# ssteinberg/wave_tracer

Hardware: AMD Instinct MI355X
Metric: Msamples/sec (whole node), cornell-box 1440^2 wave-mode (higher is better)
Workload: dtype f32

## Files before the change

### wave_tracer_amd/csrc/kernels_trace.hip

```cpp
#include "wtgpu_kernels.h"

namespace wtk {

}
#include "kernels_trace_refill.h"
namespace wtk {

__global__ void __launch_bounds__(kBlock, WTGPU_LB_TRACE) k_trace_refill(launch_args_t a, int in, int first_round, uint32_t round) { trace_refill_body(a, in, first_round, round); }

#ifndef WTGPU_SM_EXACT_MIN
#define WTGPU_SM_EXACT_MIN 24
#endif
#ifndef WTGPU_SM_SPLIT_NODE
#define WTGPU_SM_SPLIT_NODE 0
#endif
#ifndef WTGPU_SM_BOTH
#define WTGPU_SM_BOTH 0
#endif
enum : int { PH_IDLE = 0, PH_NODE = 1, PH_TRI = 2, PH_EXACT = 3, PH_SERVE = 4, PH_POLICY = 5, PH_RAYDONE = 6 };
#ifdef WTGPU_SM_PROF
#define SP_DECL() unsigned long long sp_t[8] = {0, 0, 0, 0, 0, 0, 0, 0}, sp_l[8] = {0, 0, 0, 0, 0, 0, 0, 0}, sp_n[8] = {0, 0, 0, 0, 0, 0, 0, 0}; long long sp_c = 0
#define SP_BEGIN() sp_c = clock64()
#define SP_END(i, mask) do { const long long d_ = clock64() - sp_c; sp_t[i] += (unsigned long long)d_; sp_l[i] += (unsigned long long)d_ * (unsigned long long)__popcll(mask); sp_n[i] += 1; } while (0)
#else
// ... 608 lines not shown
            uint32_t* slot = a.st.tris + (size_t)w * kTriListWords;
            const uint_list_t tris{slot, 1u, (a.collect_list & 1u) ? kMaxConeTris : 0u, reinterpret_cast<float*>(slot + kMaxConeTris)};
            cone_query_t q;
            for (;;) {
                const int need = aw_next(a.sc, ts.env, rt, stack, ts.aw, q, r);
                if (need == AW_FINAL) break;
                if (need == AW_TEST) {
                    aw_test_done(ts.aw, cone_attempt_too_short_by(a.sc, ts.env, ts.aw.cand, ts.aw.sr, ts.aw.min_df_prog));
                    continue;
                }
                while (cq_running(q)) {
                    while (q.s > 0 && q.leaf == 0) cq_node_step(ns, ts.env, stack, q);
                    if (q.leaf != 0) cq_leaf_step(a.sc, ts.env, stack, tris, q);
                }
                cq_end(ts.env, tris, q);
                if (aw_query_done(a.sc, ts.env, ts.aw, q.rec, r)) break;
            }
        }
        tr_finish(a, ctl, ctr, have, w, r);
    }
    if (a.count_stats) flush_counters(a.st.counters, ctr);
}

__global__ void __launch_bounds__(64, WTGPU_LB_HEAVY) k_trace_heavy(launch_args_t a) {
    __shared__ coop_shared_t sh;
    coop_set_dropped_counter(sh, a.st.counters + kDroppedSlot);
    uint32_t* ctl = a.st.ctl;
    const uint32_t n = ctl[CTL_HEAVY_COUNT];
    const uint32_t* hq = a.st.heavy_queue;
    uint32_t* head = ctl + CTL_HEAVY_HEAD;
    bdpt_counters_t ctr;
    memset(&ctr, 0, sizeof(ctr));
    const size_t W2 = 2 * (size_t)a.st.cap;
    const bool rt = a.sc.sensor.ray_trace_only || a.sc.opts.force_ray_tracing;
    for (;;) {
        const uint32_t item = wave_grab_item(head);
        if (item >= n) break;
        const uint32_t w = hq[item];
        const walk_trace_in_t wk = walk_load_trace_in(a.st.walks, a.st.walk_words, w);
        const uint_list_t tris{a.st.tris + (size_t)w * kTriListWords, 1u, (a.collect_list & 1u) ? kMaxConeTris : 0u};
        const cone_t env = walk_trace_envelope(a.sc, wk);
        unsigned long long prof[12] = {0, 0, 0, 0, 0, 0, 0, 0, 0, 0, 0, 0};
        const long long tt0 = a.profile == 2 ? clock64() : 0;
        const float dist0 = __uint_as_float(a.st.trav[(size_t)w * kTravWords + WT_TRAV_WORD(dist)]);
        const uint32_t seg0 = a.st.trav[(size_t)w * kTravWords + WT_TRAV_WORD(ntris)];
        const uint32_t nray0 = a.st.trav[(size_t)w * kTravWords + WT_TRAV_WORD(n_ray_queries)], ncone0 = a.st.trav[(size_t)w * kTravWords + WT_TRAV_WORD(n_cone_queries)];
        ray_hit_t axis;
        axis.tuid = a.st.trav[(size_t)w * kTravWords + WT_TRAV_WORD(tuid)];
        axis.bx = __uint_as_float(a.st.trav[(size_t)w * kTravWords + WT_TRAV_WORD(bx)]);
        axis.by = __uint_as_float(a.st.trav[(size_t)w * kTravWords + WT_TRAV_WORD(by)]);
        axis.dist = __uint_as_float(a.st.trav[(size_t)w * kTravWords + WT_TRAV_WORD(pdist)]);
        axis.front_face = a.st.trav[(size_t)w * kTravWords + WT_TRAV_WORD(front_face)];
        const uint32_t short0 = a.st.trav[(size_t)w * kTravWords + WT_TRAV_WORD(overflow)];
        const trav_result_t tr2 = coop_traverse(a.sc, env, wavenum_to_wavelen_m(wk.k), WT_INF, rt, sh, tris, a.profile == 2 ? prof : nullptr, true, seg0, dist0, nray0, ncone0,
                                                &axis, !(a.collect_list & 1u) || (a.collect_list & 2u), a.heavy_probe != 0, a.heavy_cache ? short0 : kInvalid, a.heavy_cache ? wk.prev_offset_tuid : kInvalid, a.heavy_cache != 0);
        if (a.profile == 2 && threadIdx.x == 0) {
            prof[3] = (unsigned long long)(clock64() - tt0);
            for (int q = 0; q < 4; ++q) atomicAdd(a.st.counters + kNumCounters + q, prof[q]);
            atomicAdd(a.st.counters + kNumCounters + 5, prof[5]);
            atomicAdd(a.st.counters + kNumCounters + 6, prof[6]);
            atomicAdd(a.st.counters + kNumCounters + 7, prof[7]);
            for (int q = 8; q < 12; ++q) atomicAdd(a.st.counters + kNumCounters + q, prof[q]);
            atomicAdd(a.st.counters + kNumCounters + 4, 1ull);
        }
        if (threadIdx.x == 0) {
            soa_store(a.st.trav, kTravWords, w, tr2);
            ctr.segments += 1;
            ctr.ray_queries += tr2.n_ray_queries;
            ctr.cone_queries += tr2.n_cone_queries;
            if (a.collect_list & 1u) ctr.cone_tri_overflow += tr2.overflow;
        }
    }
    if (a.count_stats) flush_counters(a.st.counters, ctr);
}

__global__ void __launch_bounds__(256) k_calib_copy(const uint32_t* in, uint32_t* out, size_t n) {
    for (size_t i = blockIdx.x * (size_t)blockDim.x + threadIdx.x; i < n; i += (size_t)gridDim.x * blockDim.x) out[i] = in[i] + 1u;
}

__global__ void __launch_bounds__(kBlock) k_trace_rays(scene_t sc, const float* rays, uint32_t n, float* dist, uint32_t* tuid, float* bary, uint32_t* front) {
    __shared__ stack_entry_t lds[kLdsStack * kBlock];
    const uint32_t i = blockIdx.x * kBlock + threadIdx.x;
    if (i >= n) return;
    stack_entry_t spill[kSpillStack];
    stack_ref_t stack;
    lds_stack(lds, spill, stack);
    const float* r = rays + 8 * (size_t)i;
    ray_hit_t h;
    ads_intersect_ray(sc, vec3{r[0], r[1], r[2]}, vec3{r[3], r[4], r[5]}, range_t{r[6], r[7]}, stack, h);
    dist[i] = h.dist;
    tuid[i] = h.tuid;
    bary[2 * i] = h.bx;
    bary[2 * i + 1] = h.by;
    front[i] = h.front_face;
}
__global__ void __launch_bounds__(kBlock) k_traverse_cones(scene_t sc, const float* cones, uint32_t n, uint32_t cap, float* dist, uint32_t* flags,
// ... 22 lines not shown
            const uint32_t v = tris[j];
            uint32_t pos = m < cap ? m : cap;
            while (pos > 0 && out_tris[(size_t)i * cap + pos - 1] > v) {
                if (pos < cap) out_tris[(size_t)i * cap + pos] = out_tris[(size_t)i * cap + pos - 1];
                --pos;
            }
            if (pos < cap) out_tris[(size_t)i * cap + pos] = v;
            if (m < cap) ++m;
        }
    }
}

__global__ void __launch_bounds__(64) k_query_regions(scene_t sc, const float* cones, uint32_t n, uint32_t edge_cap, float* dist, uint32_t* flags,
                                                      uint32_t* primary, uint32_t* ntris, uint32_t* nedges, uint32_t* edges, float* flux, unsigned long long* dropped) {
    __shared__ coop_shared_t sh;
    __shared__ coop_gather_shared_t gsh;
    __shared__ coop_edges_t eg;
    coop_set_dropped_counter(sh, dropped);
    coop_set_dropped_counter(gsh, dropped);
    const uint32_t i = blockIdx.x;
    if (i >= n) return;
    const float* c = cones + 10 * (size_t)i;
    const vec3 d = normalize(vec3{c[3], c[4], c[5]});
    const cone_t env = make_cone(vec3{c[0], c[1], c[2]}, d, build_orthogonal_frame(d).t, c[6], c[8], c[7]);
    const uint_list_t none{nullptr, 1u, 0u};
    const trav_result_t tr = coop_traverse(sc, env, c[9], WT_INF, false, sh, none, nullptr, false, 0, 0.f, 0, 0, nullptr, true);
    uint32_t prim = kInvalid;
    gather_out_t ge{0.0, 0u, 0u, 0u}, gf{0.0, 0u, 0u, 0u};
    if (tr.ballistic) {
        prim = tr.tuid;
    } else if (!tr.empty) {
        const range_t izr{tr.dist, tr.dist + tr.region_depth};
        prim = tr.tuid;
        const vec2 ax = cone_axes(env, tr.dist);
        ge = coop_gather(sc, env, izr, env, cone_frame(env), izr, vec2{1.f, 1.f}, false, gsh, false, true, nullptr, 1, &eg);
        __syncthreads();
        if (sc.n_edges <= kCoopEdgeBits) {
            ge.n_edges = coop_edge_count(sc, eg);
            coop_edge_write(sc, eg, edges + (size_t)i * edge_cap, edge_cap);
        } else
            for (uint32_t j = threadIdx.x; j < ge.n_edges && j < edge_cap; j += 64) edges[(size_t)i * edge_cap + j] = eg.edge_ids[j];
        __syncthreads();
        gf = coop_gather(sc, env, izr, env, cone_frame(env), izr, vec2{ax.x / kBeamEnvelope, ax.y / kBeamEnvelope}, tr.front_face != 0, gsh, true, false);
    }
    if (threadIdx.x == 0) {
        dist[i] = tr.dist;
        flags[i] = (tr.empty ? 1u : 0u) | (tr.ballistic ? 2u : 0u) | (tr.front_face ? 4u : 0u);
        primary[i] = prim;
        ntris[i] = gf.n_tris;
// ... 7 lines not shown
```

### wave_tracer_amd/csrc/wt/coop.h

```cpp
#pragma once
#if defined(__HIPCC__)
#include "bvh.h"
#include "gauss.h"

namespace wt {

constexpr int kCoopStack = 512;
#ifndef WTGPU_COOP_LEAF_TRIS
#define WTGPU_COOP_LEAF_TRIS 256
#endif
constexpr uint32_t kCoopLeafTris = WTGPU_COOP_LEAF_TRIS;
constexpr uint32_t kCoopGatherLeafTris = 64;
constexpr uint32_t kCoopTriBuf = 64 + 8 * kCoopLeafTris;

#ifndef WTGPU_COOP_FLUSH_AT
#define WTGPU_COOP_FLUSH_AT 12
#endif
constexpr uint32_t kCoopFlushAt = WTGPU_COOP_FLUSH_AT;
constexpr uint32_t kCoopSurvCap = 128;

#ifndef WT_COOP_SPHERES
#define WT_COOP_SPHERES 1
#endif
#ifndef WT_COOP_SPHERE_PREFETCH
// ... 9 lines not shown
    float hit_dist[64];
};
struct coop_gather_shared_t {
    unsigned long long* dropped;
    stack_entry_t stack[kCoopStack];
    uint32_t tri_buf[64 + 8 * 64];
    uint32_t surv[kCoopSurvCap];
};
struct coop_edges_t {
    uint32_t edge_ids[96];
    uint32_t edge_bits[1024];
};
constexpr uint32_t kCoopEdgeBits = 32768;

template <class SH>
WT_D void coop_set_dropped_counter(SH& sh, unsigned long long* slot) {
    if (threadIdx.x == 0) sh.dropped = slot;
    __syncthreads();
}
WT_D float wave_min(float v) {
#pragma unroll
    for (int off = 32; off > 0; off >>= 1) v = fminf(v, __shfl_xor(v, off, 64));
    return v;
}

WT_D bool cone_child_test(const bvh8_node_t& n, int i, vec3 ro, vec3 rd, vec3 rinvd, bool sx, bool sy, bool sz, float ta, float ix,
                                       const range_t& range, float& tmin_out) {
    float ominx = n.minx[i] - ro.x, ominy = n.miny[i] - ro.y, ominz = n.minz[i] - ro.z;
    float omaxx = n.maxx[i] - ro.x, omaxy = n.maxy[i] - ro.y, omaxz = n.maxz[i] - ro.z;
    const bool outside = cone_box_outside(ominx, ominy, ominz, omaxx, omaxy, omaxz, rd, ta, ix, range);
    const float bx = sx ? ominx : omaxx, by = sy ? ominy : omaxy, bz = sz ? ominz : omaxz;
    const float dot_d_b = rd.x * bx + rd.y * by + rd.z * bz;
    const float maxz = clampf(dot_d_b, 0.f, range.max);
    const float enlr = fmaf(maxz, ta, ix);
    ominx -= enlr;
    ominy -= enlr;
    ominz -= enlr;
    omaxx += enlr;
    omaxy += enlr;
    omaxz += enlr;
    const float dminx = (sx ? omaxx : ominx) * rinvd.x, dmaxx = (sx ? ominx : omaxx) * rinvd.x;
    const float dminy = (sy ? omaxy : ominy) * rinvd.y, dmaxy = (sy ? ominy : omaxy) * rinvd.y;
    const float dminz = (sz ? omaxz : ominz) * rinvd.z, dmaxz = (sz ? ominz : omaxz) * rinvd.z;
    float tmin = 0.f, tmax = dmaxx;
    tmin = fmaxf_(tmin, dminx);
    tmax = fminf_(tmax, dmaxy);
    tmin = fmaxf_(tmin, dminy);
    tmax = fminf_(tmax, dmaxz);
    tmin = fmaxf_(tmin, dminz);
    tmin_out = tmin;
    return !outside && tmin <= tmax && tmax >= range.min && tmin <= range.max && !(tmin >= range.max);
}

template <bool any_hit>
WT_D bool coop_cone_query(const scene_t& sc, const cone_t& cone, const range_t& searchrange, float z_scale, coop_shared_t& sh,
                                       const uint_list_t& tris, cone_hit_t& rec, unsigned long long* prof = nullptr, float min_progress = -WT_INF) {
    const int lane = threadIdx.x & 63;
    const int grp = lane >> 3, sub = lane & 7;
    rec.dist = WT_INF;
    rec.front_face = 0;
    rec.ntris = 0;
    rec.overflow = 0;
    rec.aborted = 0;
    rec.too_short = 0;
    rec.short_tuid = kInvalid;
    if (sc.n_nodes == 0) return false;
    const vec3 ro = cone.o, rd = cone.d;
    const vec3 rinvd{1.f / rd.x, 1.f / rd.y, 1.f / rd.z};
    const bool sx = __builtin_signbit(rinvd.x), sy = __builtin_signbit(rinvd.y), sz = __builtin_signbit(rinvd.z);
    const float ta = cone.tan_alpha, ix = cone.x0;
    range_t range = any_hit ? searchrange : cone_search_range(cone, searchrange, rec.dist, z_scale);
    float slab_max = range.max;
    int s = 1;
    uint32_t leaf_total = 0, nsurv = 0;
    if (lane == 0) sh.stack[0] = stack_entry_t{0.f, 1};
    __syncthreads();
    auto compact = [&](float zmax) __attribute__((always_inline)) {
        if (rec.ntris == 0) return;
        __syncthreads();
        const bool mine = (uint32_t)lane < rec.ntris;
        const uint32_t val = mine ? tris[lane] : 0u;
        const float dv = mine ? sh.hit_dist[lane] : 0.f;
        const bool keep = mine && !(dv > zmax);
        const unsigned long long km = __ballot(keep);
        __syncthreads();
        if (keep) {
            const uint32_t np_ = (uint32_t)__popcll(km & ((1ull << lane) - 1ull));
            tris[np_] = val;
            sh.hit_dist[np_] = dv;
        }
        rec.ntris = (uint32_t)__popcll(km);
        __syncthreads();
    };
    auto flush = [&]() __attribute__((always_inline)) -> bool {
        __syncthreads();
        bool any = false;
        for (uint32_t b2 = 0; b2 < nsurv && !any; b2 += 64) {
#ifdef WTGPU_COOP_PROF
            if (prof) prof[9] += 1;
#endif
            const uint32_t k2 = b2 + lane;
            bool hit = false, ff = false;
            float d = WT_INF;
            uint32_t t2 = 0;
            if (k2 < nsurv) {
                t2 = sh.surv[k2];
                const tri_geo_t tri = sc.tri_geo[t2];
                ff = dot(tri.n, -rd) > 0.f;
                cone_tri_hit_t ht;
                if (intersect_cone_tri<any_hit>(cone, tri.a, tri.b, tri.c, tri.n, range, ht) && !(ht.dist > range.max)) {
                    hit = true;
                    d = ht.dist;
                }
            }
            const unsigned long long mask = __ballot(hit);
            if (!mask) continue;
            if (any_hit) {
                rec.short_tuid = (uint32_t)__shfl((int)t2, __ffsll((long long)mask) - 1, 64);
                any = true;
                break;
            }
            const float dm = wave_min(d);
            if (dm < rec.dist) {
                const unsigned long long m2 = __ballot(hit && d == dm);
                const int src = __ffsll((long long)m2) - 1;
                rec.front_face = (uint32_t)__shfl((int)ff, src, 64);
                rec.dist = dm;
                if (rec.dist - searchrange.min < min_progress) {
                    rec.short_tuid = (uint32_t)__shfl((int)t2, src, 64);
                    rec.too_short = 1;
                    any = true;
                    break;
                }
                range = cone_search_range(cone, searchrange, rec.dist, z_scale);
                slab_max = range.max;
                compact(slab_max);
            }
            const bool hit2 = hit && !(d > slab_max);
            const unsigned long long mask2 = __ballot(hit2);
            const uint32_t pos = rec.ntris + (uint32_t)__popcll(mask2 & ((1ull << lane) - 1ull));
            if (hit2 && pos < tris.cap) {
                tris[pos] = t2;
                sh.hit_dist[pos & 63u] = d;
            }
            const uint32_t total = rec.ntris + (uint32_t)__popcll(mask2);
            const uint32_t newn = total < tris.cap ? total : tris.cap;
            rec.overflow += total - newn;
            rec.ntris = newn;
            if (rec.overflow > 0) range.max = fminf_(range.max, rec.dist);
        }
        nsurv = 0;
        __syncthreads();
        return any;
    };
#ifdef WTGPU_COOP_PROF
    long long cp_t = clock64();
#define CP(k)                                              \
    do {                                                   \
        const long long n_ = clock64();                    \
        if (prof) prof[k] += (unsigned long long)(n_ - cp_t); \
        cp_t = n_;                                         \
    } while (0)
#else
#define CP(k) ((void)0)
#endif
    for (;;) {
        const long long ta0 = prof ? clock64() : 0;
        while (s > 0 && leaf_total < 64u) {
            const int np = s < 8 ? s : 8;
#ifndef WTGPU_COOP_PROF
            if (prof) prof[7] += 1ull + ((unsigned long long)np << 32);
#endif
// ... 30 lines not shown
            CP(1);
            const unsigned long long hm = __ballot(h);
            if (hm) {
                const uint32_t gbits = (uint32_t)(hm >> (grp * 8)) & 0xffu;
                int rank = 0;
#pragma unroll
                for (int j = 0; j < 8; ++j) {
                    const float tj = __shfl(tmin, (lane & ~7) + j, 64);
                    if (((gbits >> j) & 1u) && (tj > tmin || (tj == tmin && j < sub))) ++rank;
                }
                const int above = grp < 7 ? __popcll(hm >> ((grp + 1) * 8)) : 0;
                const int pos = s + above + rank;
                if (h && pos < kCoopStack) sh.stack[pos] = stack_entry_t{tmin, cp};
                else if (h) atomicAdd(sh.dropped, 1ull);
                const int total = s + __popcll(hm);
                s = total < kCoopStack ? total : kCoopStack;
            }
            CP(2);
            const unsigned long long lm = __ballot(leafish && sub == 0 && cnt > 0);
            unsigned long long m = lm;
            while (m) {
                const int src = __ffsll((long long)m) - 1;
                m &= m - 1;
                uint32_t c = (uint32_t)__shfl((int)cnt, src, 64);
                const uint32_t t = (uint32_t)__shfl((int)t0, src, 64);
                if (c > kCoopLeafTris) c = kCoopLeafTris;
                for (uint32_t q = (uint32_t)lane; q < c; q += 64u) sh.tri_buf[leaf_total + q] = t + q;
                leaf_total += c;
            }
            __syncthreads();
            CP(3);
        }
        if (prof) prof[5] += (unsigned long long)(clock64() - ta0);
        const long long tb0 = prof ? clock64() : 0;
        bool found_any = false;
#ifdef WTGPU_COOP_PROF
        if (prof) { prof[10] += 1; prof[11] += leaf_total; prof[8] += (leaf_total + 63u) / 64u; }
#endif
#if WT_COOP_SPHERES
        {
            const float4* spheres = coop_tri_spheres(sc);
            uint32_t n2 = 0;
            for (uint32_t base0 = 0; base0 < leaf_total; base0 += 64u * kCoopSpherePrefetch) {
                float4 bs[kCoopSpherePrefetch];
                uint32_t tu[kCoopSpherePrefetch];
#pragma unroll
                for (uint32_t j = 0; j < kCoopSpherePrefetch; ++j) {
                    const uint32_t k = base0 + 64u * j + lane;
// ... 7 lines not shown
#pragma unroll
                for (uint32_t j = 0; j < kCoopSpherePrefetch; ++j) asm volatile("" : "+v"(bs[j].x), "+v"(bs[j].y), "+v"(bs[j].z), "+v"(bs[j].w));
                __syncthreads();
#pragma unroll
                for (uint32_t j = 0; j < kCoopSpherePrefetch; ++j) {
                    const uint32_t k = base0 + 64u * j + lane;
                    const bool p1 = k < leaf_total && cone_sphere_maybe(cone, vec3{bs[j].x, bs[j].y, bs[j].z}, bs[j].w, range);
                    const unsigned long long pm1 = __ballot(p1);
                    if (p1) sh.tri_buf[n2 + (uint32_t)__popcll(pm1 & ((1ull << lane) - 1ull))] = tu[j];
                    n2 += (uint32_t)__popcll(pm1);
                }
            }
            leaf_total = n2;
            __syncthreads();
            CP(7);
        }
#endif
        for (uint32_t base = 0; base < leaf_total && !found_any; base += 64) {
            const uint32_t k = base + lane;
            bool pass = false;
            uint32_t tuid = 0;
            if (k < leaf_total) {
                tuid = sh.tri_buf[k];
                const tri_geo_t tri = sc.tri_geo[tuid];
                pass = cone_tri_maybe(cone, tri.a, tri.b, tri.c, range);
            }
            const unsigned long long pm = __ballot(pass);
            if (pm) {
                const uint32_t pos = nsurv + (uint32_t)__popcll(pm & ((1ull << lane) - 1ull));
                if (pass && pos < kCoopSurvCap) sh.surv[pos] = tuid;
                nsurv += (uint32_t)__popcll(pm);
            }
            CP(7);
            if (nsurv >= 64u) found_any = flush();
            CP(6);
        }
        leaf_total = 0;
        CP(7);
        if (!found_any && nsurv > 0 && (s == 0 || nsurv >= kCoopFlushAt)) found_any = flush();
        CP(6);
        __syncthreads();
        if (prof) prof[6] += (unsigned long long)(clock64() - tb0);
        if (found_any && (any_hit || rec.too_short)) return true;
        if (s == 0) break;
    }
    return rec.ntris > 0;
}

// ... 257 lines not shown
        float tmin = 0.f;
        if (grp < np) {
            const bvh8_node_t& node = sc.nodes[e.ptr - 1];
            cp = node.child[sub];
            if (cp != 0 && cone_child_test(node, sub, ro, rd, rinvd, sx, sy, sz, ta, ix, slab, tmin)) {
                if (cp < 0 || sc.nodes[cp - 1].tris_count <= max_tris)
                    emit(cp);
                else
                    push = true;
            }
        }
        const unsigned long long hm = __ballot(push);
        if (hm) {
            const int pos = s + __popcll(hm & ((1ull << lane) - 1ull));
            if (push && pos < kCoopStack) sh.stack[pos] = stack_entry_t{tmin, cp};
            else if (push) emit(cp);
            const int total = s + __popcll(hm);
            s = total < kCoopStack ? total : kCoopStack;
        }
        __syncthreads();
    }
}

WT_D bool coop_ray_query(const scene_t& sc, vec3 ro, vec3 rd, const range_t& range, coop_shared_t& sh, ray_hit_t& rec) {
    const int lane = threadIdx.x & 63;
    const int grp = lane >> 3, sub = lane & 7;
    rec.dist = WT_INF;
    rec.tuid = kInvalid;
    rec.bx = rec.by = 0.f;
    rec.front_face = 0;
    if (sc.n_nodes == 0) return false;
    const vec3 rinvd{1.f / rd.x, 1.f / rd.y, 1.f / rd.z};
    const bool sx = __builtin_signbit(rinvd.x), sy = __builtin_signbit(rinvd.y), sz = __builtin_signbit(rinvd.z);
    int s = 1;
    uint32_t leaf_total = 0;
    if (lane == 0) sh.stack[0] = stack_entry_t{0.f, 1};
    __syncthreads();
    for (;;) {
        while (s > 0 && leaf_total < 64u) {
            const int np = s < 8 ? s : 8;
            stack_entry_t e{0.f, 0};
            if (grp < np) e = sh.stack[s - 1 - grp];
            s -= np;
            __syncthreads();
            const bool live = grp < np && e.t < rec.dist;
            bool leafish = false, h = false;
            uint32_t t0 = 0, cnt = 0;
            float tmin = 0.f;
            int32_t cp = 0;
            if (live) {
                if (e.ptr < 0) {
                    const bvh8_leaf_t leaf = bvh_leaf_of(e.ptr);
                    t0 = leaf.tris_ptr;
                    cnt = leaf.count;
                    leafish = true;
// ... 24 lines not shown
                }
            }
            const unsigned long long hm = __ballot(h);
            if (hm) {
                const uint32_t gbits = (uint32_t)(hm >> (grp * 8)) & 0xffu;
                int rank = 0;
#pragma unroll
                for (int j = 0; j < 8; ++j) {
                    const float tj = __shfl(tmin, (lane & ~7) + j, 64);
                    if (((gbits >> j) & 1u) && (tj > tmin || (tj == tmin && j < sub))) ++rank;
                }
                const int above = grp < 7 ? __popcll(hm >> ((grp + 1) * 8)) : 0;
                const int pos = s + above + rank;
                if (h && pos < kCoopStack) sh.stack[pos] = stack_entry_t{tmin, cp};
                else if (h) atomicAdd(sh.dropped, 1ull);
                const int total = s + __popcll(hm);
                s = total < kCoopStack ? total : kCoopStack;
            }
            const unsigned long long lm = __ballot(leafish && sub == 0 && cnt > 0);
            unsigned long long m = lm;
            while (m) {
                const int src = __ffsll((long long)m) - 1;
                m &= m - 1;
                uint32_t c = (uint32_t)__shfl((int)cnt, src, 64);
                const uint32_t t = (uint32_t)__shfl((int)t0, src, 64);
                if (c > kCoopLeafTris) c = kCoopLeafTris;
                for (uint32_t q = (uint32_t)lane; q < c; q += 64u) sh.tri_buf[leaf_total + q] = t + q;
                leaf_total += c;
            }
            __syncthreads();
        }
        if (leaf_total == 0) {
            if (s == 0) break;
            continue;
        }
        for (uint32_t base = 0; base < leaf_total; base += 64) {
            const uint32_t k = base + lane;
            bool hit = false;
            float d = WT_INF;
            uint32_t tuid = 0;
            ray_tri_hit_t ht{WT_INF, 0.f, 0.f};
            bool ff = false;
            if (k < leaf_total) {
                tuid = sh.tri_buf[k];
                const tri_geo_t tri = sc.tri_geo[tuid];
                if (intersect_ray_tri_wide(ro, rd, tri.a, tri.b, tri.c, range, ht) && ht.dist < rec.dist) {
                    hit = true;
                    d = ht.dist;
                    ff = dot(tri.n, rd) <= 0.f;
                }
            }
            const unsigned long long mask = __ballot(hit);
            if (mask) {
                const float dm = wave_min(d);
                const unsigned long long m2 = __ballot(hit && d == dm);
                const int src = __ffsll((long long)m2) - 1;
                rec.dist = dm;
                rec.tuid = (uint32_t)__shfl((int)tuid, src, 64);
                rec.bx = __shfl(ht.bx, src, 64);
                rec.by = __shfl(ht.by, src, 64);
                rec.front_face = (uint32_t)__shfl((int)ff, src, 64);
            }
        }
        leaf_total = 0;
        __syncthreads();
        if (s == 0) break;
    }
    if (!finitef(rec.dist) || rec.dist > range.max) {
        rec.dist = WT_INF;
        return false;
    }
    return true;
}

WT_D trav_result_t coop_traverse(const scene_t& sc, const cone_t& envelope, float lambda_m, float distance, bool force_ray_tracing,
                                              coop_shared_t& sh, const uint_list_t& tris, unsigned long long* prof = nullptr, bool resume = false,
                                              uint32_t seg0 = 0, float dist0 = 0.f, uint32_t nray0 = 0, uint32_t ncone0 = 0, const ray_hit_t* axis = nullptr,
                                              bool primary_always = false, bool probe_resumed = true, uint32_t short_tuid = kInvalid,
                                              uint32_t origin_tuid = kInvalid, bool use_cache = true) {
#ifdef WTGPU_COOP_PROF
#define WT_COOP_PROF(i, t0_)
#else
#define WT_COOP_PROF(i, t0_) \
    if (prof) prof[i] += (unsigned long long)(clock64() - (t0_));
#endif
    trav_result_t r;
    r.aborted = 0;
    r.origin = envelope.o;
    r.empty = 1;
    r.ballistic = 1;
    r.dist = -WT_INF;
    r.region_depth = 0.f;
    r.front_face = 0;
    r.tuid = kInvalid;
    r.bx = r.by = 0.f;
    r.pdist = 0.f;
    r.ntris = 0;
    r.overflow = 0;
    r.n_ray_queries = resume ? nray0 : 0u;
    r.n_cone_queries = resume ? ncone0 : 0u;
    const vec3 ro = envelope.o, rd = envelope.d;
    ray_hit_t ah;
    bool axis_hit;
    if (axis) {
        ah = *axis;
        axis_hit = ah.tuid != kInvalid;
    } else {
        r.n_ray_queries++;
        const long long tq0 = prof ? clock64() : 0;
        axis_hit = coop_ray_query(sc, ro, rd, range_t{0.f, distance}, sh, ah);
        WT_COOP_PROF(0, tq0)
    }
    auto ballistic_hit = [&]() __attribute__((always_inline)) {
        r.empty = 0;
        r.dist = ah.dist;
        r.tuid = ah.tuid;
        r.bx = ah.bx;
        r.by = ah.by;
        r.front_face = ah.front_face;
        r.ntris = 1;
    };
    if (force_ray_tracing || cone_is_ray(envelope)) {
        if (axis_hit) ballistic_hit();
        return r;
    }
    float dist = resume ? dist0 : 0.f;
    for (uint32_t seg = resume ? seg0 : 0u;; ++seg) {
        const float ballistic_dist = max_ballistic_distance(lambda_m, seg, 0.f);
        if (!(resume && seg == seg0)) {
            if (axis_hit && ah.dist <= fminf_(distance, dist + ballistic_dist * kBallisticScale)) {
                ballistic_hit();
                return r;
            }
            dist += ballistic_dist;
            if (ballistic_dist == WT_INF || dist >= distance) return r;
        }
        const float min_df_prog = cone_axes(envelope, dist).x / 2.f;
        cone_hit_t ch;
        r.n_cone_queries++;
        const long long tp0 = prof ? clock64() : 0;
        const range_t thin{dist, fminf_(distance, dist + min_df_prog)};
        bool near_hit = false;
        for (int c = 0; c < 2 && !near_hit; ++c) {
            const uint32_t cand = c == 0 ? short_tuid : origin_tuid;
            if (!use_cache || cand == kInvalid || (c == 1 && cand == short_tuid)) continue;
            const tri_geo_t tri = sc.tri_geo[cand];
            cone_tri_hit_t ht;
            near_hit = intersect_cone_tri<true>(envelope, tri.a, tri.b, tri.c, tri.n, thin, ht) && !(ht.dist > thin.max);
        }
        if (!near_hit) {
            uint32_t hit_tuid = kInvalid;
            near_hit = (probe_resumed || !(resume && seg == seg0)) && coop_cone_any(sc, envelope, thin, sh, prof, &hit_tuid);
            if (near_hit) short_tuid = hit_tuid;
        }
        WT_COOP_PROF(1, tp0)
        if (near_hit) continue;
        const long long tc0 = prof ? clock64() : 0;
        const float cone_max = axis_hit ? fminf_(distance, cone_axis_bound(envelope, ah.dist)) : distance;
        coop_cone(sc, envelope, range_t{dist, cone_max}, kMajorAxisToZScale, sh, tris, ch, prof, min_df_prog);
        WT_COOP_PROF(2, tc0)
        if (ch.too_short) {
            short_tuid = ch.short_tuid;
            continue;
        }
        const bool df_empty = ch.ntris == 0 && ch.overflow == 0;
        if (df_empty || ch.dist - dist >= min_df_prog) {
            r.ballistic = 0;
            r.empty = df_empty;
            r.dist = df_empty ? -WT_INF : ch.dist;
            r.front_face = ch.front_face;
            r.ntris = ch.ntris;
            r.overflow = ch.overflow;
            r.region_depth = df_empty ? 0.f : kMajorAxisToZScale * cone_axes(envelope, ch.dist).x;
            if (!df_empty && (primary_always || ch.overflow > 0)) primary_from_axis(sc, envelope, axis_hit, ah, r);
            return r;
        }
    }
}

}
#endif
// ... 1 lines not shown
```

### wave_tracer_amd/csrc/wtgpu.hip

```cpp
#include "wtgpu_host.h"

thread_local std::string g_err;

static void note_rounds(wtgpu_scene* s, uint32_t n) { s->rounds_hist[s->rounds_hist_n++ % 8u] = n; }
static int drain_rec(wtgpu_scene* s, chunk_rec_t& r) {
    if (!r.busy) return WTGPU_OK;
    HIP_CHECK(hipEventSynchronize(r.ev[r.ev_final]));
    const uint32_t rounds = r.h_ctl[CTL_ROUNDS];
    s->cap_hits += r.h_ctl[CTL_COUNT0 + (r.rounds_launched & 1u)] + r.h_ctl[CTL_BACK0 + (r.rounds_launched & 1u)];
    s->acc[4] += rounds;
    s->acc[5] += rounds;
    s->acc[6] += 1;
    s->rounds_launched_total += r.rounds_launched;
    if (s->knobs.timing) {
        auto elapsed = [](hipEvent_t a, hipEvent_t b) {
            float ms = 0.f;
            return hipEventElapsedTime(&ms, a, b) == hipSuccess ? ms : 0.f;
        };
        s->acc[0] += elapsed(r.ev[0], r.ev[1]);
        size_t e = 1;
        for (uint32_t k = 0; k < r.rounds_timed; ++k, e += 6) {
            static const int slot[6] = {1, 7, 2, 8, 9, 10};
            for (int q = 0; q < 6; ++q) s->acc[slot[q]] += elapsed(r.ev[e + q], r.ev[e + q + 1]);
        }
// ... 79 lines not shown
                s->ev_stagger_last = r.ev_stagger;
            }
            uint32_t g0, gh;
            if (K.decay_q > 0) {
                const double f = std::min(1.0, (double)K.decay_c * std::pow(K.decay_q * .01, (double)round));
                g0 = std::max<uint32_t>(2u, (uint32_t)(gf * f));
                gh = std::max<uint32_t>(2u, (uint32_t)(std::min<uint32_t>(grid_heavy, walks_per_sample * nb) * f));
            } else {
                const uint32_t shrink = round < K.shrink_r1 ? 1u : (round < K.shrink_r2 ? K.shrink_f1 : K.shrink_f2);
                g0 = std::max<uint32_t>(1u, gf / shrink);
                gh = std::max<uint32_t>(1u, std::min<uint32_t>(grid_heavy, walks_per_sample * nb) / (round < K.shrink_r1 ? 1u : (round < K.shrink_r2 ? K.shrink_h1 : 32u)));
            }
            const int sf = round == r_begin ? stage_from : 0;
            if (sf <= 0 && dbg_stage >= 2 + 3 * (int)round) {
                if (round < K.trace_ab) {
                    const int rc = trace_ab_round(s, a, st_, in, first, round, g0);
                    if (rc) return rc;
                } else if (K.trace_sm || (K.trace_staged && round < K.trace_staged_rounds))
                    launch_trace_alt(s, a, st_, in, first, round, g0);
                else
                    HP_LAUNCH(k_trace_refill, dim3(g0), dim3(kBlock), 0, st_, a, in, first, round);
            }
            rec(r, st_);
            if (sf <= 1 && dbg_stage >= 3 + 3 * (int)round) HP_LAUNCH(k_trace_heavy, dim3(gh), dim3(64), 0, st_, a);
            rec(r, st_);
            if (path_mode) {
                if (round > 0) HP_LAUNCH(k_path_fsd, dim3(gh), dim3(64), 0, st_, a, ps, round);
                if (dbg_stage >= 4 + 3 * (int)round) HP_LAUNCH(k_path_interact, dim3(g0), dim3(kBlock), 0, st_, a, ps, in, first, round);
                HP_LAUNCH(k_path_edges, dim3(gh), dim3(64), 0, st_, a, ps);
                HP_LAUNCH(k_path_interact_b, dim3(std::max<uint32_t>(1u, g0 / 2u)), dim3(kBlock), 0, st_, a, ps, in, round);
                HP_LAUNCH(k_path_nee, dim3(gh), dim3(64), 0, st_, a, ps, round);
                rec(r, st_);
                rec(r, st_);
                rec(r, st_);
                rec(r, st_);
                continue;
            }
            if (sf > 2) {
            } else if (K.sorted_interact) {
                HP_LAUNCH(k_classify, dim3(g0), dim3(kBlock), 0, st_, a, in, first);
                if (K.sorted_interact >= 2)
                    HP_LAUNCH(k_interact_sorted, dim3(g0), dim3(kBlock), 0, st_, a, in);
                else {
                HP_LAUNCH(k_interact_diffuse, dim3(std::max<uint32_t>(1u, g0 / K.grid_div_cls[0])), dim3(kBlock), 0, st_, a, in);
                HP_LAUNCH(k_interact_dielectric, dim3(std::max<uint32_t>(1u, g0 / K.grid_div_cls[1])), dim3(kBlock), 0, st_, a, in);
                HP_LAUNCH(k_interact_spm, dim3(std::max<uint32_t>(1u, g0 / K.grid_div_cls[2])), dim3(kBlock), 0, st_, a, in);
                HP_LAUNCH(k_interact_any, dim3(std::max<uint32_t>(1u, g0 / K.grid_div_cls[3])), dim3(kBlock), 0, st_, a, in);
// ... 282 lines not shown
```

### wave_tracer_amd/csrc/wtgpu_kernels.h

```cpp
#pragma once
#include <hip/hip_runtime.h>

#include <cstddef>
#include <cstdint>
#include <cstring>

#include "../../include/wtgpu.h"
#include "wt/bdpt.h"
#include "wt/coop.h"
#include "wt/coop_fsd.h"
#include "wt/coop_utd.h"
#include "wt/path.h"

using namespace wt;
namespace wt {
struct tonemap_args_t;
}

namespace wtk {


#ifndef WTGPU_LB_TRACE
#define WTGPU_LB_TRACE 3
#endif
#ifndef WTGPU_LB_HEAVY
#define WTGPU_LB_HEAVY 2
#endif
#ifndef WTGPU_LB_INTERACT
#define WTGPU_LB_INTERACT 3
#endif
#ifndef WTGPU_LB_INTERACT_B
#define WTGPU_LB_INTERACT_B 3
#endif
#ifndef WTGPU_LB_INTERACT_C
#define WTGPU_LB_INTERACT_C 3
#endif
#ifndef WTGPU_LB_FLUX
#define WTGPU_LB_FLUX 3
#endif
#ifndef WTGPU_LB_CONNECT
#define WTGPU_LB_CONNECT 2
#endif
constexpr uint32_t kFluxTaskTris = 2048;
constexpr int kBlock = 128;
#ifndef WTGPU_LDS_STACK
#define WTGPU_LDS_STACK 20
#endif
constexpr int kLdsStack = WTGPU_LDS_STACK;
constexpr uint32_t kConeBudget = 96;
// ... 223 lines not shown
            uint32_t* dst = base + (size_t)__builtin_amdgcn_readlane(idx, r) * stride + __builtin_amdgcn_readlane(off, r);
#pragma unroll
            for (int w0 = 0; w0 < W; w0 += 64)
                if (w0 + lane < W) dst[w0 + lane] = lds[(r & 31) * P + w0 + lane];
        }
        __builtin_amdgcn_wave_barrier();
    }
}

constexpr uint32_t kFlushGrid = 64;
constexpr int kEnumBlock = 1024;
constexpr uint32_t kSplatCols = kBlock + 2;
#ifndef WTGPU_HARD_BLOCK
#define WTGPU_HARD_BLOCK 256
#endif
__global__ void k_generate(launch_args_t a);
__global__ void k_trace_refill(launch_args_t a, int in, int first_round, uint32_t round);
__global__ void k_trace_sm(launch_args_t a, int in, int first_round, uint32_t round);
__global__ void k_tr_axis(launch_args_t a, int in, int first_round, uint32_t round);
__global__ void k_tr_cone(launch_args_t a, uint32_t it);
__global__ void k_tr_policy(launch_args_t a, uint32_t it);
__global__ void k_tr_tail(launch_args_t a, uint32_t it);
__global__ void k_trace_heavy(launch_args_t a);
__global__ void k_interact(launch_args_t a, int in, int first_round);
__global__ void k_classify(launch_args_t a, int in, int first_round);
__global__ void k_interact_diffuse(launch_args_t a, int in);
__global__ void k_interact_dielectric(launch_args_t a, int in);
__global__ void k_interact_spm(launch_args_t a, int in);
__global__ void k_interact_any(launch_args_t a, int in);
__global__ void k_interact_sorted(launch_args_t a, int in);
__global__ void k_interact_coop(launch_args_t a, int in, int first_round);
__global__ void k_edges(launch_args_t a);
__global__ void k_interact_b(launch_args_t a, int in);
__global__ void k_light_rounds(launch_args_t a, int in, uint32_t round, uint32_t max_rounds);
__global__ void k_flux_split(launch_args_t a);
__global__ void k_flux_tasks(launch_args_t a);
__global__ void k_interact_c(launch_args_t a, int in);
__global__ void k_interact_c_hard(launch_args_t a, int in);
__global__ void k_path_generate(launch_args_t a);
__global__ void k_path_fsd(launch_args_t a, const path_state_t* __restrict__ ps, uint32_t round);
__global__ void k_path_edges(launch_args_t a, const path_state_t* __restrict__ ps);
__global__ void k_path_interact(launch_args_t a, const path_state_t* __restrict__ ps, int in, int first_round, uint32_t round);
__global__ void k_path_interact_b(launch_args_t a, const path_state_t* __restrict__ ps, int in, uint32_t round);
__global__ void k_path_nee(launch_args_t a, const path_state_t* __restrict__ ps, uint32_t round);
__global__ void k_path_flush(launch_args_t a, int in);
__global__ void k_connect_enum(launch_args_t a);
// ... 44 lines not shown
```

Before: 30.61.

## Scalarize wave-uniform values in cooperative traversal and split heavy kernel profiling

Wraps wave-uniform traversal state (cone envelope, ranges, shuffled hit results, per-walk trav words) in readfirstlane so the compiler can keep it in scalar registers and cut vector register pressure. The heavy trace kernel is templated so the profiling path compiles into a separate kernel, its per-thread counter struct becomes four scalars flushed with atomics, and its launch-bounds occupancy hint rises from 2 to 3. Triangle vertices are now read as float4 loads. The risk is spilling if the higher occupancy target forces register limits, plus correctness depending on the values really being uniform.

```diff
diff --git a/wave_tracer_amd/csrc/kernels_trace.hip b/wave_tracer_amd/csrc/kernels_trace.hip
--- a/wave_tracer_amd/csrc/kernels_trace.hip
+++ b/wave_tracer_amd/csrc/kernels_trace.hip
@@ -654,39 +654,39 @@
     if (a.count_stats) flush_counters(a.st.counters, ctr);
 }
 
-__global__ void __launch_bounds__(64, WTGPU_LB_HEAVY) k_trace_heavy(launch_args_t a) {
-    __shared__ coop_shared_t sh;
+template <bool PROF>
+WT_D void trace_heavy_body(const launch_args_t& a, coop_shared_t& sh) {
     coop_set_dropped_counter(sh, a.st.counters + kDroppedSlot);
     uint32_t* ctl = a.st.ctl;
     const uint32_t n = ctl[CTL_HEAVY_COUNT];
     const uint32_t* hq = a.st.heavy_queue;
     uint32_t* head = ctl + CTL_HEAVY_HEAD;
-    bdpt_counters_t ctr;
-    memset(&ctr, 0, sizeof(ctr));
-    const size_t W2 = 2 * (size_t)a.st.cap;
+    unsigned long long n_segments = 0, n_ray_queries = 0, n_cone_queries = 0, n_overflow = 0;
     const bool rt = a.sc.sensor.ray_trace_only || a.sc.opts.force_ray_tracing;
     for (;;) {
         const uint32_t item = wave_grab_item(head);
         if (item >= n) break;
-        const uint32_t w = hq[item];
+        const uint32_t w = uniform(hq[item]);
         const walk_trace_in_t wk = walk_load_trace_in(a.st.walks, a.st.walk_words, w);
         const uint_list_t tris{a.st.tris + (size_t)w * kTriListWords, 1u, (a.collect_list & 1u) ? kMaxConeTris : 0u};
-        const cone_t env = walk_trace_envelope(a.sc, wk);
+        const cone_t env = uniform(walk_trace_envelope(a.sc, wk));
         unsigned long long prof[12] = {0, 0, 0, 0, 0, 0, 0, 0, 0, 0, 0, 0};
-        const long long tt0 = a.profile == 2 ? clock64() : 0;
-        const float dist0 = __uint_as_float(a.st.trav[(size_t)w * kTravWords + WT_TRAV_WORD(dist)]);
-        const uint32_t seg0 = a.st.trav[(size_t)w * kTravWords + WT_TRAV_WORD(ntris)];
-        const uint32_t nray0 = a.st.trav[(size_t)w * kTravWords + WT_TRAV_WORD(n_ray_queries)], ncone0 = a.st.trav[(size_t)w * kTravWords + WT_TRAV_WORD(n_cone_queries)];
+        const long long tt0 = PROF ? clock64() : 0;
+        const uint32_t* tv = a.st.trav + (size_t)w * kTravWords;
+        const float dist0 = uniform(__uint_as_float(tv[WT_TRAV_WORD(dist)]));
+        const uint32_t seg0 = uniform(tv[WT_TRAV_WORD(ntris)]);
+        const uint32_t nray0 = uniform(tv[WT_TRAV_WORD(n_ray_queries)]), ncone0 = uniform(tv[WT_TRAV_WORD(n_cone_queries)]);
         ray_hit_t axis;
-        axis.tuid = a.st.trav[(size_t)w * kTravWords + WT_TRAV_WORD(tuid)];
-        axis.bx = __uint_as_float(a.st.trav[(size_t)w * kTravWords + WT_TRAV_WORD(bx)]);
-        axis.by = __uint_as_float(a.st.trav[(size_t)w * kTravWords + WT_TRAV_WORD(by)]);
-        axis.dist = __uint_as_float(a.st.trav[(size_t)w * kTravWords + WT_TRAV_WORD(pdist)]);
-        axis.front_face = a.st.trav[(size_t)w * kTravWords + WT_TRAV_WORD(front_face)];
-        const uint32_t short0 = a.st.trav[(size_t)w * kTravWords + WT_TRAV_WORD(overflow)];
-        const trav_result_t tr2 = coop_traverse(a.sc, env, wavenum_to_wavelen_m(wk.k), WT_INF, rt, sh, tris, a.profile == 2 ? prof : nullptr, true, seg0, dist0, nray0, ncone0,
-                                                &axis, !(a.collect_list & 1u) || (a.collect_list & 2u), a.heavy_probe != 0, a.heavy_cache ? short0 : kInvalid, a.heavy_cache ? wk.prev_offset_tuid : kInvalid, a.heavy_cache != 0);
-        if (a.profile == 2 && threadIdx.x == 0) {
+        axis.tuid = uniform(tv[WT_TRAV_WORD(tuid)]);
+        axis.bx = uniform(__uint_as_float(tv[WT_TRAV_WORD(bx)]));
+        axis.by = uniform(__uint_as_float(tv[WT_TRAV_WORD(by)]));
+        axis.dist = uniform(__uint_as_float(tv[WT_TRAV_WORD(pdist)]));
+        axis.front_face = uniform(tv[WT_TRAV_WORD(front_face)]);
+        const uint32_t short0 = uniform(tv[WT_TRAV_WORD(overflow)]);
+        const uint32_t origin0 = uniform(wk.prev_offset_tuid);
+        const trav_result_t tr2 = coop_traverse(a.sc, env, uniform(wavenum_to_wavelen_m(wk.k)), WT_INF, rt, sh, tris, PROF ? prof : nullptr, true, seg0, dist0, nray0, ncone0,
+                                                &axis, !(a.collect_list & 1u) || (a.collect_list & 2u), a.heavy_probe != 0, a.heavy_cache ? short0 : kInvalid, a.heavy_cache ? origin0 : kInvalid, a.heavy_cache != 0);
+        if (PROF && threadIdx.x == 0) {
             prof[3] = (unsigned long long)(clock64() - tt0);
             for (int q = 0; q < 4; ++q) atomicAdd(a.st.counters + kNumCounters + q, prof[q]);
             atomicAdd(a.st.counters + kNumCounters + 5, prof[5]);
@@ -695,15 +695,27 @@
             for (int q = 8; q < 12; ++q) atomicAdd(a.st.counters + kNumCounters + q, prof[q]);
             atomicAdd(a.st.counters + kNumCounters + 4, 1ull);
         }
-        if (threadIdx.x == 0) {
-            soa_store(a.st.trav, kTravWords, w, tr2);
-            ctr.segments += 1;
-            ctr.ray_queries += tr2.n_ray_queries;
-            ctr.cone_queries += tr2.n_cone_queries;
-            if (a.collect_list & 1u) ctr.cone_tri_overflow += tr2.overflow;
-        }
-    }
-    if (a.count_stats) flush_counters(a.st.counters, ctr);
+        n_segments += 1;
+        n_ray_queries += tr2.n_ray_queries;
+        n_cone_queries += tr2.n_cone_queries;
+        if (a.collect_list & 1u) n_overflow += tr2.overflow;
+        if (threadIdx.x == 0) soa_store(a.st.trav, kTravWords, w, tr2);
+    }
+    if (a.count_stats && threadIdx.x == 0) {
+        unsigned long long* g = a.st.counters;
+        if (n_segments) atomicAdd(g + offsetof(bdpt_counters_t, segments) / 8, n_segments);
+        if (n_ray_queries) atomicAdd(g + offsetof(bdpt_counters_t, ray_queries) / 8, n_ray_queries);
+        if (n_cone_queries) atomicAdd(g + offsetof(bdpt_counters_t, cone_queries) / 8, n_cone_queries);
+        if (n_overflow) atomicAdd(g + offsetof(bdpt_counters_t, cone_tri_overflow) / 8, n_overflow);
+    }
+}
+__global__ void __launch_bounds__(64, WTGPU_LB_HEAVY) k_trace_heavy(launch_args_t a) {
+    __shared__ coop_shared_t sh;
+    trace_heavy_body<false>(a, sh);
+}
+__global__ void __launch_bounds__(64, 2) k_trace_heavy_prof(launch_args_t a) {
+    __shared__ coop_shared_t sh;
+    trace_heavy_body<true>(a, sh);
 }
 
 __global__ void __launch_bounds__(256) k_calib_copy(const uint32_t* in, uint32_t* out, size_t n) {
@@ -772,9 +784,9 @@
     if (i >= n) return;
     const float* c = cones + 10 * (size_t)i;
     const vec3 d = normalize(vec3{c[3], c[4], c[5]});
-    const cone_t env = make_cone(vec3{c[0], c[1], c[2]}, d, build_orthogonal_frame(d).t, c[6], c[8], c[7]);
+    const cone_t env = uniform(make_cone(vec3{c[0], c[1], c[2]}, d, build_orthogonal_frame(d).t, c[6], c[8], c[7]));
     const uint_list_t none{nullptr, 1u, 0u};
-    const trav_result_t tr = coop_traverse(sc, env, c[9], WT_INF, false, sh, none, nullptr, false, 0, 0.f, 0, 0, nullptr, true);
+    const trav_result_t tr = coop_traverse(sc, env, uniform(c[9]), WT_INF, false, sh, none, nullptr, false, 0, 0.f, 0, 0, nullptr, true);
     uint32_t prim = kInvalid;
     gather_out_t ge{0.0, 0u, 0u, 0u}, gf{0.0, 0u, 0u, 0u};
     if (tr.ballistic) {
diff --git a/wave_tracer_amd/csrc/wt/coop.h b/wave_tracer_amd/csrc/wt/coop.h
--- a/wave_tracer_amd/csrc/wt/coop.h
+++ b/wave_tracer_amd/csrc/wt/coop.h
@@ -55,6 +55,33 @@
 #pragma unroll
     for (int off = 32; off > 0; off >>= 1) v = fminf(v, __shfl_xor(v, off, 64));
     return v;
+}
+WT_D int uniform(int x) { return __builtin_amdgcn_readfirstlane(x); }
+WT_D uint32_t uniform(uint32_t x) { return (uint32_t)__builtin_amdgcn_readfirstlane((int)x); }
+WT_D bool uniform(bool x) { return __builtin_amdgcn_readfirstlane((int)x) != 0; }
+WT_D float uniform(float x) { return __int_as_float(__builtin_amdgcn_readfirstlane(__float_as_int(x))); }
+WT_D vec3 uniform(vec3 v) { return vec3{uniform(v.x), uniform(v.y), uniform(v.z)}; }
+WT_D range_t uniform(const range_t& r) { return range_t{uniform(r.min), uniform(r.max)}; }
+WT_D cone_t uniform(const cone_t& c) {
+    cone_t u;
+    u.o = uniform(c.o);
+    u.d = uniform(c.d);
+    u.x = uniform(c.x);
+    u.x0 = uniform(c.x0);
+    u.tan_alpha = uniform(c.tan_alpha);
+    u.e = uniform(c.e);
+    u.one_over_e = uniform(c.one_over_e);
+    u.z_apex = uniform(c.z_apex);
+    return u;
+}
+
+WT_D void coop_tri_vertices(const scene_t& sc, uint32_t tuid, vec3& a, vec3& b, vec3& c) {
+    const float4* q = reinterpret_cast<const float4*>(sc.tri_geo + tuid);
+    const float4 q0 = q[0], q1 = q[1];
+    const float q2 = reinterpret_cast<const float*>(q)[8];
+    a = vec3{q0.x, q0.y, q0.z};
+    b = vec3{q0.w, q1.x, q1.y};
+    c = vec3{q1.z, q1.w, q2};
 }
 
 WT_D bool cone_child_test(const bvh8_node_t& n, int i, vec3 ro, vec3 rd, vec3 rinvd, bool sx, bool sy, bool sz, float ta, float ix,
@@ -86,8 +113,11 @@
 }
 
 template <bool any_hit>
-WT_D bool coop_cone_query(const scene_t& sc, const cone_t& cone, const range_t& searchrange, float z_scale, coop_shared_t& sh,
-                                       const uint_list_t& tris, cone_hit_t& rec, unsigned long long* prof = nullptr, float min_progress = -WT_INF) {
+WT_D bool coop_cone_query(const scene_t& sc, const cone_t& cone_, const range_t& searchrange_, float z_scale, coop_shared_t& sh,
+                                       const uint_list_t& tris, cone_hit_t& rec, unsigned long long* prof = nullptr, float min_progress_ = -WT_INF) {
+    const cone_t cone = uniform(cone_);
+    const range_t searchrange = uniform(searchrange_);
+    const float min_progress = uniform(min_progress_);
     const int lane = threadIdx.x & 63;
     const int grp = lane >> 3, sub = lane & 7;
     rec.dist = WT_INF;
@@ -99,10 +129,10 @@
     rec.short_tuid = kInvalid;
     if (sc.n_nodes == 0) return false;
     const vec3 ro = cone.o, rd = cone.d;
-    const vec3 rinvd{1.f / rd.x, 1.f / rd.y, 1.f / rd.z};
+    const vec3 rinvd = uniform(vec3{1.f / rd.x, 1.f / rd.y, 1.f / rd.z});
     const bool sx = __builtin_signbit(rinvd.x), sy = __builtin_signbit(rinvd.y), sz = __builtin_signbit(rinvd.z);
     const float ta = cone.tan_alpha, ix = cone.x0;
-    range_t range = any_hit ? searchrange : cone_search_range(cone, searchrange, rec.dist, z_scale);
+    range_t range = any_hit ? searchrange : uniform(cone_search_range(cone, searchrange, rec.dist, z_scale));
     float slab_max = range.max;
     int s = 1;
     uint32_t leaf_total = 0, nsurv = 0;
@@ -149,23 +179,23 @@
             const unsigned long long mask = __ballot(hit);
             if (!mask) continue;
             if (any_hit) {
-                rec.short_tuid = (uint32_t)__shfl((int)t2, __ffsll((long long)mask) - 1, 64);
+                rec.short_tuid = uniform((uint32_t)__shfl((int)t2, __ffsll((long long)mask) - 1, 64));
                 any = true;
                 break;
             }
-            const float dm = wave_min(d);
+            const float dm = uniform(wave_min(d));
             if (dm < rec.dist) {
                 const unsigned long long m2 = __ballot(hit && d == dm);
                 const int src = __ffsll((long long)m2) - 1;
-                rec.front_face = (uint32_t)__shfl((int)ff, src, 64);
+                rec.front_face = uniform((uint32_t)__shfl((int)ff, src, 64));
                 rec.dist = dm;
                 if (rec.dist - searchrange.min < min_progress) {
-                    rec.short_tuid = (uint32_t)__shfl((int)t2, src, 64);
+                    rec.short_tuid = uniform((uint32_t)__shfl((int)t2, src, 64));
                     rec.too_short = 1;
                     any = true;
                     break;
                 }
-                range = cone_search_range(cone, searchrange, rec.dist, z_scale);
+                range = uniform(cone_search_range(cone, searchrange, rec.dist, z_scale));
                 slab_max = range.max;
                 compact(slab_max);
             }
@@ -180,7 +210,7 @@
             const uint32_t newn = total < tris.cap ? total : tris.cap;
             rec.overflow += total - newn;
             rec.ntris = newn;
-            if (rec.overflow > 0) range.max = fminf_(range.max, rec.dist);
+            if (rec.overflow > 0) range.max = uniform(fminf_(range.max, rec.dist));
         }
         nsurv = 0;
         __syncthreads();
@@ -257,8 +287,8 @@
             while (m) {
                 const int src = __ffsll((long long)m) - 1;
                 m &= m - 1;
-                uint32_t c = (uint32_t)__shfl((int)cnt, src, 64);
-                const uint32_t t = (uint32_t)__shfl((int)t0, src, 64);
+                uint32_t c = uniform((uint32_t)__shfl((int)cnt, src, 64));
+                const uint32_t t = uniform((uint32_t)__shfl((int)t0, src, 64));
                 if (c > kCoopLeafTris) c = kCoopLeafTris;
                 for (uint32_t q = (uint32_t)lane; q < c; q += 64u) sh.tri_buf[leaf_total + q] = t + q;
                 leaf_total += c;
@@ -312,8 +342,9 @@
             uint32_t tuid = 0;
             if (k < leaf_total) {
                 tuid = sh.tri_buf[k];
-                const tri_geo_t tri = sc.tri_geo[tuid];
-                pass = cone_tri_maybe(cone, tri.a, tri.b, tri.c, range);
+                vec3 va, vb, vc;
+                coop_tri_vertices(sc, tuid, va, vb, vc);
+                pass = cone_tri_maybe(cone, va, vb, vc, range);
             }
             const unsigned long long pm = __ballot(pass);
             if (pm) {
@@ -617,7 +648,9 @@
     }
 }
 
-WT_D bool coop_ray_query(const scene_t& sc, vec3 ro, vec3 rd, const range_t& range, coop_shared_t& sh, ray_hit_t& rec) {
+WT_D bool coop_ray_query(const scene_t& sc, vec3 ro_, vec3 rd_, const range_t& range_, coop_shared_t& sh, ray_hit_t& rec) {
+    const vec3 ro = uniform(ro_), rd = uniform(rd_);
+    const range_t range = uniform(range_);
     const int lane = threadIdx.x & 63;
     const int grp = lane >> 3, sub = lane & 7;
     rec.dist = WT_INF;
@@ -625,7 +658,7 @@
     rec.bx = rec.by = 0.f;
     rec.front_face = 0;
     if (sc.n_nodes == 0) return false;
-    const vec3 rinvd{1.f / rd.x, 1.f / rd.y, 1.f / rd.z};
+    const vec3 rinvd = uniform(vec3{1.f / rd.x, 1.f / rd.y, 1.f / rd.z});
     const bool sx = __builtin_signbit(rinvd.x), sy = __builtin_signbit(rinvd.y), sz = __builtin_signbit(rinvd.z);
     int s = 1;
     uint32_t leaf_total = 0;
@@ -696,8 +729,8 @@
             while (m) {
                 const int src = __ffsll((long long)m) - 1;
                 m &= m - 1;
-                uint32_t c = (uint32_t)__shfl((int)cnt, src, 64);
-                const uint32_t t = (uint32_t)__shfl((int)t0, src, 64);
+                uint32_t c = uniform((uint32_t)__shfl((int)cnt, src, 64));
+                const uint32_t t = uniform((uint32_t)__shfl((int)t0, src, 64));
                 if (c > kCoopLeafTris) c = kCoopLeafTris;
                 for (uint32_t q = (uint32_t)lane; q < c; q += 64u) sh.tri_buf[leaf_total + q] = t + q;
                 leaf_total += c;
@@ -726,14 +759,14 @@
             }
             const unsigned long long mask = __ballot(hit);
             if (mask) {
-                const float dm = wave_min(d);
+                const float dm = uniform(wave_min(d));
                 const unsigned long long m2 = __ballot(hit && d == dm);
                 const int src = __ffsll((long long)m2) - 1;
                 rec.dist = dm;
-                rec.tuid = (uint32_t)__shfl((int)tuid, src, 64);
-                rec.bx = __shfl(ht.bx, src, 64);
-                rec.by = __shfl(ht.by, src, 64);
-                rec.front_face = (uint32_t)__shfl((int)ff, src, 64);
+                rec.tuid = uniform((uint32_t)__shfl((int)tuid, src, 64));
+                rec.bx = uniform(__shfl(ht.bx, src, 64));
+                rec.by = uniform(__shfl(ht.by, src, 64));
+                rec.front_face = uniform((uint32_t)__shfl((int)ff, src, 64));
             }
         }
         leaf_total = 0;
@@ -747,11 +780,15 @@
     return true;
 }
 
-WT_D trav_result_t coop_traverse(const scene_t& sc, const cone_t& envelope, float lambda_m, float distance, bool force_ray_tracing,
+WT_D trav_result_t coop_traverse(const scene_t& sc, const cone_t& envelope_, float lambda_m_, float distance_, bool force_ray_tracing,
                                               coop_shared_t& sh, const uint_list_t& tris, unsigned long long* prof = nullptr, bool resume = false,
-                                              uint32_t seg0 = 0, float dist0 = 0.f, uint32_t nray0 = 0, uint32_t ncone0 = 0, const ray_hit_t* axis = nullptr,
-                                              bool primary_always = false, bool probe_resumed = true, uint32_t short_tuid = kInvalid,
-                                              uint32_t origin_tuid = kInvalid, bool use_cache = true) {
+                                              uint32_t seg0_ = 0, float dist0 = 0.f, uint32_t nray0 = 0, uint32_t ncone0 = 0, const ray_hit_t* axis = nullptr,
+                                              bool primary_always = false, bool probe_resumed = true, uint32_t short_tuid_ = kInvalid,
+                                              uint32_t origin_tuid_ = kInvalid, bool use_cache = true) {
+    const cone_t envelope = uniform(envelope_);
+    const float lambda_m = uniform(lambda_m_), distance = uniform(distance_);
+    const uint32_t seg0 = uniform(seg0_), origin_tuid = uniform(origin_tuid_);
+    uint32_t short_tuid = uniform(short_tuid_);
 #ifdef WTGPU_COOP_PROF
 #define WT_COOP_PROF(i, t0_)
 #else
@@ -771,13 +808,17 @@
     r.pdist = 0.f;
     r.ntris = 0;
     r.overflow = 0;
-    r.n_ray_queries = resume ? nray0 : 0u;
-    r.n_cone_queries = resume ? ncone0 : 0u;
+    r.n_ray_queries = resume ? uniform(nray0) : 0u;
+    r.n_cone_queries = resume ? uniform(ncone0) : 0u;
     const vec3 ro = envelope.o, rd = envelope.d;
     ray_hit_t ah;
     bool axis_hit;
     if (axis) {
-        ah = *axis;
+        ah.dist = uniform(axis->dist);
+        ah.tuid = uniform(axis->tuid);
+        ah.bx = uniform(axis->bx);
+        ah.by = uniform(axis->by);
+        ah.front_face = uniform(axis->front_face);
         axis_hit = ah.tuid != kInvalid;
     } else {
         r.n_ray_queries++;
@@ -798,22 +839,22 @@
         if (axis_hit) ballistic_hit();
         return r;
     }
-    float dist = resume ? dist0 : 0.f;
+    float dist = resume ? uniform(dist0) : 0.f;
     for (uint32_t seg = resume ? seg0 : 0u;; ++seg) {
-        const float ballistic_dist = max_ballistic_distance(lambda_m, seg, 0.f);
+        const float ballistic_dist = uniform(max_ballistic_distance(lambda_m, seg, 0.f));
         if (!(resume && seg == seg0)) {
             if (axis_hit && ah.dist <= fminf_(distance, dist + ballistic_dist * kBallisticScale)) {
                 ballistic_hit();
                 return r;
             }
-            dist += ballistic_dist;
+            dist = uniform(dist + ballistic_dist);
             if (ballistic_dist == WT_INF || dist >= distance) return r;
         }
-        const float min_df_prog = cone_axes(envelope, dist).x / 2.f;
+        const float min_df_prog = uniform(cone_axes(envelope, dist).x / 2.f);
         cone_hit_t ch;
         r.n_cone_queries++;
         const long long tp0 = prof ? clock64() : 0;
-        const range_t thin{dist, fminf_(distance, dist + min_df_prog)};
+        const range_t thin{dist, uniform(fminf_(distance, dist + min_df_prog))};
         bool near_hit = false;
         for (int c = 0; c < 2 && !near_hit; ++c) {
             const uint32_t cand = c == 0 ? short_tuid : origin_tuid;
@@ -830,7 +871,7 @@
         WT_COOP_PROF(1, tp0)
         if (near_hit) continue;
         const long long tc0 = prof ? clock64() : 0;
-        const float cone_max = axis_hit ? fminf_(distance, cone_axis_bound(envelope, ah.dist)) : distance;
+        const float cone_max = axis_hit ? uniform(fminf_(distance, cone_axis_bound(envelope, ah.dist))) : distance;
         coop_cone(sc, envelope, range_t{dist, cone_max}, kMajorAxisToZScale, sh, tris, ch, prof, min_df_prog);
         WT_COOP_PROF(2, tc0)
         if (ch.too_short) {
diff --git a/wave_tracer_amd/csrc/wtgpu.hip b/wave_tracer_amd/csrc/wtgpu.hip
--- a/wave_tracer_amd/csrc/wtgpu.hip
+++ b/wave_tracer_amd/csrc/wtgpu.hip
@@ -125,7 +125,12 @@
                     HP_LAUNCH(k_trace_refill, dim3(g0), dim3(kBlock), 0, st_, a, in, first, round);
             }
             rec(r, st_);
-            if (sf <= 1 && dbg_stage >= 3 + 3 * (int)round) HP_LAUNCH(k_trace_heavy, dim3(gh), dim3(64), 0, st_, a);
+            if (sf <= 1 && dbg_stage >= 3 + 3 * (int)round) {
+                if (a.profile == 2)
+                    HP_LAUNCH(k_trace_heavy_prof, dim3(gh), dim3(64), 0, st_, a);
+                else
+                    HP_LAUNCH(k_trace_heavy, dim3(gh), dim3(64), 0, st_, a);
+            }
             rec(r, st_);
             if (path_mode) {
                 if (round > 0) HP_LAUNCH(k_path_fsd, dim3(gh), dim3(64), 0, st_, a, ps, round);
diff --git a/wave_tracer_amd/csrc/wtgpu_kernels.h b/wave_tracer_amd/csrc/wtgpu_kernels.h
--- a/wave_tracer_amd/csrc/wtgpu_kernels.h
+++ b/wave_tracer_amd/csrc/wtgpu_kernels.h
@@ -24,7 +24,7 @@
 #define WTGPU_LB_TRACE 3
 #endif
 #ifndef WTGPU_LB_HEAVY
-#define WTGPU_LB_HEAVY 2
+#define WTGPU_LB_HEAVY 3
 #endif
 #ifndef WTGPU_LB_INTERACT
 #define WTGPU_LB_INTERACT 3
@@ -294,6 +294,7 @@
 __global__ void k_tr_policy(launch_args_t a, uint32_t it);
 __global__ void k_tr_tail(launch_args_t a, uint32_t it);
 __global__ void k_trace_heavy(launch_args_t a);
+__global__ void k_trace_heavy_prof(launch_args_t a);
 __global__ void k_interact(launch_args_t a, int in, int first_round);
 __global__ void k_classify(launch_args_t a, int in, int first_round);
 __global__ void k_interact_diffuse(launch_args_t a, int in);
```

Result: faster. 32.10 (median of 6 runs) (+4.9%).
